# CyrilMorel42/LZ4-JPEG

Hardware: AMD Instinct MI355X
Metric: LZ4 compress GB/s + JPEG DCT Mpixel/s at 1/2/4/8 MI355X; % HBM roofline (higher is better)
Workload: dtype u8

## Files before the change

lz4-jpeg_amd/csrc/lz4r_emit.h:

```cpp
#pragma once
#include "lz4r_layout.h"
#include "wave64.h"

namespace {

constexpr int kGH = 32;
constexpr int kEW = 8;
constexpr int kRecPre = kHeadW;
constexpr int kGSplit = kGT / kGH;
constexpr int kEmitImg = kGH * kBlkOutMax + 32;
constexpr int kStagePad = 16;
constexpr int kStage = kStagePad + kGH * kBlk + 32;
static_assert(kStage < (1 << 16), "stage offsets fit 16 bits");

__device__ __forceinline__ void or_bytes(uint32_t *buf32, int x, uint32_t v) {
  const uint64_t w = (uint64_t)v << (8 * (x & 3));
  atomicOr(&buf32[x >> 2], (uint32_t)w);
  atomicOr(&buf32[(x >> 2) + 1], (uint32_t)(w >> 32));
}

__device__ __forceinline__ void emit_records(const int wv, const int lane, const int h0,
                                             const int h1, const uint64_t G0, const int lead,
                                             const uint64_t *toff, uint8_t *img,
                                             const uint8_t *stage,
                                             const uint32_t (*recst)[kRecPre],
                                             uint32_t (*marks)[64], const uint4 *pmask,
                                             const uint8_t *__restrict__ wovf) {
  {
    constexpr int kBW = kGH / kEW;
    const int bl0 = h0 + wv * kBW, bl1 = min(h1, bl0 + kBW);
    if (bl0 < bl1) {
      uint32_t *const out32 = reinterpret_cast<uint32_t *>(img);
      const int nbk = bl1 - bl0;
      const uint32_t hd = lane < nbk ? recst[bl0 - h0 + lane][0] : 0u;
      const uint32_t ns = hd >> 16;
      const uint32_t sinc = wave_incl_add(ns);
      const int Stot = (int)lane63(sinc);
      const int sst = (int)(sinc - ns);
      int st[kBW];
#pragma unroll
      for (int i = 0; i < kBW; ++i)
        st[i] = i < nbk ? __builtin_amdgcn_readlane(sst, i) : 0x7fffffff;
      int end_prev = 0, wcur = lead + (int)(toff[bl0] - G0) + 3;
      for (int f0 = 0; f0 < Stot; f0 += 64) {
        const int f = f0 + lane;
        const bool valid = f < Stot;
        int bi = 0, sb = 0;
#pragma unroll
        for (int i = 1; i < kBW; ++i) {
          const bool ge = f >= st[i];
          bi += ge ? 1 : 0;
          sb = ge ? st[i] : sb;
        }
        const int k = f - sb;
        const int hb = bl0 + bi;
        const uint32_t *rp = reinterpret_cast<const uint32_t *>(wovf + (hb - h0) * kOvf);
        const uint32_t r =
            !valid ? 0u : (1 + k < kRecPre ? recst[hb - h0][1 + k] : rp[1 + k - kRecPre]);
        const int M = (int)((r >> 9) & 255u), D = (int)(r & 511u);
        const int end = (int)(r >> 19);
        const int cpos = end - M;
        const uint32_t upv = dpp<0x138, 0xf, 0xf>((uint32_t)end);
        const int pend = k == 0 ? 0 : (lane == 0 ? end_prev : (int)upv);
        end_prev = (int)lane63((uint32_t)end);
        const int L = cpos - pend;
        const int rem = (L - 15) & 255;
        const int le = L >= 15 ? (rem == 255 ? 2 : 1) : 0;
        const int mx = (M - 4) & 255;
        const bool mextW = M >= 4 && mx >= 15, mextS = M != 0 && mx >= 15;
        const int bytes = valid ? 5 + le + L + (mextW ? 1 : 0) : 0;
        const uint32_t inc = wave_incl_add((uint32_t)bytes);
        const int o = wcur + 3 * bi + (int)inc - bytes;
        const int ib = o - 3;
        const int ol = o + 3 + le;
        if (valid) {
          const int tl = L >= 15 ? 15 : L;
          const int tm = M == 0 ? 0 : (M >= 19 ? 15 : mx);
          const uint32_t ext = le == 0 ? 0u : (rem == 255 ? 255u : (uint32_t)rem);
          const uint32_t SZ = (uint32_t)(5 + le + L + (mextS ? 1 : 0));
          or_bytes(out32, o, (uint32_t)((tl << 4) | tm) | (SZ << 8) | (ext << 24));
          or_bytes(out32, ol + L, (uint32_t)D | (mextW ? ((uint32_t)(mx - 15) & 255u) << 16 : 0u));
          if (k == 0) {
            const uint32_t bh = recst[hb - h0][0];
            or_bytes(out32, ib, ((bh >> 16) & 255u) | ((((bh & 0xFFFFu) + 3u) & 0xFFFFu) << 8));
          }
        }
        {
          const int cw = valid && L > 0 ? ((ol + L - 1) >> 4) - (ol >> 4) + 1 : 0;
          const uint32_t cinc = wave_incl_add((uint32_t)cw);
          const int C = (int)lane63(cinc);
          const int stw = (int)dpp<0x138, 0xf, 0xf>(cinc);
          const int src = kStagePad + kBlk * (hb - h0) + pend;
          const uint32_t rw = ((uint32_t)((ol >> 4) - stw) & 0xFFFFu) | ((uint32_t)(src - ol) << 16);
          const uint32_t rb = (uint32_t)ol | ((uint32_t)(ol + L) << 16);
          uint32_t carry = 0;
          for (int w0 = 0; w0 < C; w0 += 64) {
            wave_sync();
            marks[wv][lane] = 0u;
            if (cw > 0 && stw >= w0 && stw < w0 + 64) marks[wv][stw - w0] = (uint32_t)lane + 1u;
            wave_sync();
            const uint32_t k1 = max(wave_incl_max(marks[wv][lane]), carry);
            carry = lane63(k1);
            const int gw = w0 + lane;
            const int kr = ((int)k1 - 1) & 63;
            const uint32_t kw = (uint32_t)__shfl((int)rw, kr, 64);
            const uint32_t kb = (uint32_t)__shfl((int)rb, kr, 64);
            if (gw < C) {
              const int t = 16 * ((int)(int16_t)(kw & 0xFFFFu) + gw);
              const int xs = t + ((int)kw >> 16);
              const uint32_t *iw = reinterpret_cast<const uint32_t *>(stage + (xs & ~3));
              const uint32_t d0 = iw[0], d1 = iw[1], d2 = iw[2], d3 = iw[3], d4 = iw[4];
              const uint32_t sh = (uint32_t)xs & 3u;
              const int lb = max((int)(kb & 0xFFFFu) - t, 0), hb = min((int)(kb >> 16) - t, 16);
              const uint4 ml = pmask[lb], mh = pmask[hb];
              const uint32_t v0 = __builtin_amdgcn_alignbyte(d1, d0, sh) & (ml.x ^ mh.x);
              const uint32_t v1 = __builtin_amdgcn_alignbyte(d2, d1, sh) & (ml.y ^ mh.y);
              const uint32_t v2 = __builtin_amdgcn_alignbyte(d3, d2, sh) & (ml.z ^ mh.z);
              const uint32_t v3 = __builtin_amdgcn_alignbyte(d4, d3, sh) & (ml.w ^ mh.w);
              atomicOr(reinterpret_cast<unsigned long long *>(img + t),
                       (unsigned long long)v1 << 32 | v0);
              atomicOr(reinterpret_cast<unsigned long long *>(img + t + 8),
                       (unsigned long long)v3 << 32 | v2);
            }
          }
        }
        wcur += (int)lane63(inc);
      }
    }
  }
}

__device__ __forceinline__ void emit_store(const int tid, const int wv, const int lane,
                                           const uint64_t G0, const uint64_t G1, const int lead,
                                           const uint8_t *img, uint8_t *__restrict__ out) {
  if (G1 <= G0) return;
  const uint64_t F = G0 - (uint64_t)lead;
  uint8_t *const outF = out + F;
  const uint32_t nrel = (uint32_t)(G1 - F);
  const uint32_t c0 = lead ? 1u : 0u, c1 = nrel >> 4;
  for (uint32_t ci = c0 + (uint32_t)tid; ci < c1; ci += 64 * kEW)
    __builtin_nontemporal_store(reinterpret_cast<const u32x4 *>(img)[ci],
                                reinterpret_cast<u32x4 *>(outF + 16u * ci));
  if (wv == kEW - 1 && lane < 32) {
    const uint32_t x = lane < 16 ? (uint32_t)lane : 16u * c1 + (uint32_t)(lane - 16);
    const bool own = lane < 16 ? (c0 && x >= (uint32_t)lead && x < nrel) : (c1 >= c0 && x < nrel);
    if (own) outF[x] = img[x];
  }
}

__global__ __launch_bounds__(64 * kEW) void lz4_emit(
    const uint8_t *__restrict__ in, const uint8_t *__restrict__ heads,
    const uint8_t *__restrict__ ovfs, size_t slot_base,
    const uint32_t *__restrict__ tsz, size_t ntiles, size_t g_first,
    const uint32_t *__restrict__ gsum, const uint64_t *__restrict__ part,
    uint8_t *__restrict__ out, uint64_t cap, int hdr, uint64_t nb_total, uint32_t last_n,
    uint64_t *__restrict__ boff) {
  __shared__ uint64_t toff[kGT + 1];
  __shared__ alignas(16) uint8_t img[kEmitImg];
  __shared__ alignas(16) uint8_t stage[kStage];
  __shared__ uint32_t marks[kEW][64];
  __shared__ uint4 pmask[17];
  __shared__ uint32_t recst[kGH][kRecPre];
  const int tid = threadIdx.x, lane = tid & 63, wv = tid >> 6;
  const uint32_t nwg = (uint32_t)((ntiles - g_first * kGT + kGT - 1) / kGT) * kGSplit;
  const uint32_t per = (nwg + 7) / 8;
  const uint32_t wg = (blockIdx.x & 7u) * per + (blockIdx.x >> 3);
  if (wg >= nwg) return;
  const size_t g = g_first + wg / kGSplit;
  const int h0 = (int)(wg % kGSplit) * kGH;
  const size_t g0 = g * kGT;
  const int nt = (int)min((size_t)kGT, ntiles - g0);
  if (h0 >= nt) return;
  const int h1 = min(nt, h0 + kGH);
  const size_t b0 = g0 + h0;
  const int len = (h1 - h0 - 1) * kBlk + (g0 + h1 == nb_total ? (int)last_n : kBlk);
  const uint8_t *src = in + b0 * kBlk;
  const bool al16 = ((uintptr_t)src & 15) == 0;
  const int n16 = al16 ? len >> 4 : 0;
  uint64_t pt = 0;
  uint32_t gs = 0, tv = 0;
  if (tid < 64) {
    __builtin_amdgcn_s_setprio(3);
    const size_t p = g0 / kPart;
    const size_t gfirst = p * 64;
    gs = (gfirst + tid < g) ? gsum[gfirst + tid] : 0u;
    pt = part[p];
    tv = tid < nt ? tsz[g0 + tid] : 0u;
  }
  constexpr int kPerSlot = kRecPre / 4;
  static_assert(kGH * kPerSlot <= 64 * kEW, "one record load per thread");
  uint4 rv = make_uint4(0, 0, 0, 0);
  const int rhb = tid / kPerSlot, rj = tid % kPerSlot;
  const uint8_t *const wheads = heads + (b0 - slot_base) * (size_t)kHead;
  const uint8_t *const wovf = ovfs + (b0 - slot_base) * (size_t)kOvf;
  if (tid < (h1 - h0) * kPerSlot) {
    const u32x4 t = __builtin_nontemporal_load(reinterpret_cast<const u32x4 *>(wheads) + tid);
    rv = make_uint4(t.x, t.y, t.z, t.w);
  }
  constexpr int kSt16 = (kGH * kBlk) / 16;
  constexpr int kStPer = (kSt16 + 64 * kEW - 1) / (64 * kEW);
  uint4 sv[kStPer];
#pragma unroll
  for (int k = 0; k < kStPer; ++k) {
    const int i = tid + k * 64 * kEW;
    u32x4 t = {0u, 0u, 0u, 0u};
    if (i < n16) t = __builtin_nontemporal_load(reinterpret_cast<const u32x4 *>(src) + i);
    sv[k] = make_uint4(t.x, t.y, t.z, t.w);
  }
  for (int i = tid; i < kEmitImg / 16; i += 64 * kEW)
    reinterpret_cast<uint4 *>(img)[i] = make_uint4(0, 0, 0, 0);
  if (tid < 64) {
    const uint64_t base = pt + lane63(wave_incl_add(gs));
    const uint32_t inc = wave_incl_add(tv);
    toff[tid] = base + inc - tv;
    if (tid == 63) toff[kGT] = base + inc;
    if (h0 == 0 && tid < nt) boff[g0 + tid] = base + inc - tv - (uint64_t)hdr;
  }
  if (hdr && g == 0 && h0 == 0 && tid == 0 && cap > 0) out[0] = (uint8_t)nb_total;
  if (tid < (h1 - h0) * kPerSlot) reinterpret_cast<uint4 *>(&recst[rhb][0])[rj] = rv;
  if (tid < 17) {
    uint32_t m[4];
#pragma unroll
    for (int j = 0; j < 4; ++j) {
      const int n = min(max(tid - 4 * j, 0), 4);
      m[j] = n == 4 ? ~0u : (1u << (8 * n)) - 1u;
    }
    pmask[tid] = make_uint4(m[0], m[1], m[2], m[3]);
  }
  {
    uint8_t *dst = stage + kStagePad;
#pragma unroll
    for (int k = 0; k < kStPer; ++k) {
      const int i = tid + k * 64 * kEW;
      if (i < n16) reinterpret_cast<uint4 *>(dst)[i] = sv[k];
    }
    for (int i = (n16 << 4) + tid; i < len; i += 64 * kEW) dst[i] = src[i];
  }
  __syncthreads();
  __builtin_amdgcn_s_setprio(0);
  const uint64_t G0 = toff[h0];
  const int lead = (int)(((uintptr_t)out + G0) & 15);
  emit_records(wv, lane, h0, h1, G0, lead, toff, img, stage, recst, marks, pmask, wovf);
  __syncthreads();
  emit_store(tid, wv, lane, G0, min(toff[h1], cap), lead, img, out);
}

}
```

Before: 458.6.

## Distribute LZ4 emit sequences across waves by 64-sequence chunks instead of blocks

Emission work used to be split as a fixed group of blocks per wave, with each wave walking its blocks' sequences serially. Now all waves share the global sequence index space and stride over 64-sequence chunks. Each chunk finds its starting block with a ballot/popcount and works out its output offset from the block offset table, plus the chunk's tail prefix. The goal is to balance load when sequence counts differ across blocks. In exchange it adds per-chunk descriptor lookup, marks-based segmenting, and a fallback serial prefix loop for long blocks, which could cost extra work.

```diff
diff --git a/lz4-jpeg_amd/csrc/lz4r_emit.h b/lz4-jpeg_amd/csrc/lz4r_emit.h
--- a/lz4-jpeg_amd/csrc/lz4r_emit.h
+++ b/lz4-jpeg_amd/csrc/lz4r_emit.h
@@ -19,6 +19,20 @@
   atomicOr(&buf32[(x >> 2) + 1], (uint32_t)(w >> 32));
 }
 
+__device__ __forceinline__ uint32_t load_record(const uint32_t (*recst)[kRecPre],
+                                                const uint8_t *__restrict__ wovf, int b, int k) {
+  const uint32_t *rp = reinterpret_cast<const uint32_t *>(wovf + b * kOvf);
+  return 1 + k < kRecPre ? recst[b][1 + k] : rp[1 + k - kRecPre];
+}
+
+__device__ __forceinline__ int sequence_bytes(uint32_t r, int pend) {
+  const int M = (int)((r >> 9) & 255u);
+  const int L = (int)(r >> 19) - M - pend;
+  const int le = L >= 15 ? ((((L - 15) & 255) == 255) ? 2 : 1) : 0;
+  const int mx = (M - 4) & 255;
+  return 5 + le + L + (M >= 4 && mx >= 15 ? 1 : 0);
+}
+
 __device__ __forceinline__ void emit_records(const int wv, const int lane, const int h0,
                                              const int h1, const uint64_t G0, const int lead,
                                              const uint64_t *toff, uint8_t *img,
@@ -26,105 +40,118 @@
                                              const uint32_t (*recst)[kRecPre],
                                              uint32_t (*marks)[64], const uint4 *pmask,
                                              const uint8_t *__restrict__ wovf) {
-  {
-    constexpr int kBW = kGH / kEW;
-    const int bl0 = h0 + wv * kBW, bl1 = min(h1, bl0 + kBW);
-    if (bl0 < bl1) {
-      uint32_t *const out32 = reinterpret_cast<uint32_t *>(img);
-      const int nbk = bl1 - bl0;
-      const uint32_t hd = lane < nbk ? recst[bl0 - h0 + lane][0] : 0u;
-      const uint32_t ns = hd >> 16;
-      const uint32_t sinc = wave_incl_add(ns);
-      const int Stot = (int)lane63(sinc);
-      const int sst = (int)(sinc - ns);
-      int st[kBW];
-#pragma unroll
-      for (int i = 0; i < kBW; ++i)
-        st[i] = i < nbk ? __builtin_amdgcn_readlane(sst, i) : 0x7fffffff;
-      int end_prev = 0, wcur = lead + (int)(toff[bl0] - G0) + 3;
-      for (int f0 = 0; f0 < Stot; f0 += 64) {
-        const int f = f0 + lane;
-        const bool valid = f < Stot;
-        int bi = 0, sb = 0;
-#pragma unroll
-        for (int i = 1; i < kBW; ++i) {
-          const bool ge = f >= st[i];
-          bi += ge ? 1 : 0;
-          sb = ge ? st[i] : sb;
+  uint32_t *const out32 = reinterpret_cast<uint32_t *>(img);
+  const uint32_t ns = lane < h1 - h0 ? recst[lane][0] >> 16 : 0u;
+  const uint32_t sinc = wave_incl_add(ns);
+  const int T = (int)lane63(sinc);
+  const uint32_t sst = sinc - ns;
+  const uint32_t desc = ns ? ((uint32_t)(lane + 1) << 16) | sst : 0u;
+  const int rel = lead - (int)(uint32_t)G0;
+  const int wvu = __builtin_amdgcn_readfirstlane(wv);
+  const uint32_t *const toff32 = reinterpret_cast<const uint32_t *>(toff);
+  for (int f0 = 64 * wvu; f0 < T; f0 += 64 * kEW) {
+    const bool valid = f0 + lane < T;
+    const int cb = __builtin_popcountll(ballot(sst <= (uint32_t)f0)) - 1;
+    const uint32_t cd = (uint32_t)__builtin_amdgcn_readlane((int)desc, cb);
+    const int k0 = f0 - (int)(cd & 0xFFFFu);
+    const int cn = __builtin_amdgcn_readlane((int)sinc, cb) - f0;
+    const int nz = k0 != 0 ? 1 : 0;
+    const uint32_t tb = toff32[2 * (h0 + cb + nz)];
+    uint32_t rprev = recst[cb][min(k0, kRecPre - 1)];
+    wave_sync();
+    marks[wv][lane] = 0u;
+    if (sst - (uint32_t)f0 - 1u < 63u) marks[wv][sst - (uint32_t)f0] = desc;
+    wave_sync();
+    const uint32_t bd = max(wave_incl_max(marks[wv][lane]), cd);
+    const int bi = (int)(bd >> 16) - 1;
+    const int k = f0 + lane - (int)(bd & 0xFFFFu);
+    const int hb = h0 + bi;
+    uint32_t r = recst[bi][min(1 + k, kRecPre - 1)];
+    if (valid && 1 + k >= kRecPre)
+      r = reinterpret_cast<const uint32_t *>(wovf + bi * kOvf)[1 + k - kRecPre];
+    r = valid ? r : 0u;
+    asm volatile("" : "+v"(rprev));
+    if (lane == 0 && k0 >= kRecPre)
+      rprev = reinterpret_cast<const uint32_t *>(wovf + cb * kOvf)[k0 - kRecPre];
+    const int end_prev = k0 != 0 ? (int)(rprev >> 19) : 0;
+    const int M = (int)((r >> 9) & 255u), D = (int)(r & 511u);
+    const int end = (int)(r >> 19);
+    const int cpos = end - M;
+    const uint32_t upv = dpp<0x138, 0xf, 0xf>((uint32_t)end);
+    const int pend = k == 0 ? 0 : (lane == 0 ? end_prev : (int)upv);
+    const int L = cpos - pend;
+    const int rem = (L - 15) & 255;
+    const int le = L >= 15 ? (rem == 255 ? 2 : 1) : 0;
+    const int mx = (M - 4) & 255;
+    const bool mextW = M >= 4 && mx >= 15, mextS = M != 0 && mx >= 15;
+    const int bytes = valid ? 5 + le + L + (mextW ? 1 : 0) : 0;
+    const uint32_t inc = wave_incl_add((uint32_t)bytes);
+    const int tail = __builtin_amdgcn_readlane((int)inc, (cn - 1) & 63);
+    int first = rel + (int)tb + (nz ? -tail : 3);
+    if (nz & (cn > 64 ? 1 : 0)) {
+      int pre = 0, pe = 0;
+      for (int j0 = 0; j0 < k0; j0 += 64) {
+        const int j = j0 + lane;
+        const uint32_t q = j < k0 ? load_record(recst, wovf, cb, j) : 0u;
+        const uint32_t up = dpp<0x138, 0xf, 0xf>(q >> 19);
+        const int qb = j < k0 ? sequence_bytes(q, lane == 0 ? pe : (int)up) : 0;
+        pe = (int)lane63(q >> 19);
+        pre += (int)lane63(wave_incl_add((uint32_t)qb));
+      }
+      first = rel + (int)toff32[2 * (h0 + cb)] + 3 + pre;
+    }
+    const int o = first + 3 * (bi - cb) + (int)inc - bytes;
+    const int ib = o - 3;
+    const int ol = o + 3 + le;
+    if (valid) {
+      const int tl = L >= 15 ? 15 : L;
+      const int tm = M == 0 ? 0 : (M >= 19 ? 15 : mx);
+      const uint32_t ext = le == 0 ? 0u : (rem == 255 ? 255u : (uint32_t)rem);
+      const uint32_t SZ = (uint32_t)(5 + le + L + (mextS ? 1 : 0));
+      or_bytes(out32, o, (uint32_t)((tl << 4) | tm) | (SZ << 8) | (ext << 24));
+      or_bytes(out32, ol + L, (uint32_t)D | (mextW ? ((uint32_t)(mx - 15) & 255u) << 16 : 0u));
+      if (k == 0) {
+        const uint32_t bh = recst[hb - h0][0];
+        or_bytes(out32, ib, ((bh >> 16) & 255u) | ((((bh & 0xFFFFu) + 3u) & 0xFFFFu) << 8));
+      }
+    }
+    {
+      const int cw = valid && L > 0 ? ((ol + L - 1) >> 4) - (ol >> 4) + 1 : 0;
+      const uint32_t cinc = wave_incl_add((uint32_t)cw);
+      const int C = (int)lane63(cinc);
+      const int stw = (int)dpp<0x138, 0xf, 0xf>(cinc);
+      const int src = kStagePad + kBlk * (hb - h0) + pend;
+      const uint32_t rw = ((uint32_t)((ol >> 4) - stw) & 0xFFFFu) | ((uint32_t)(src - ol) << 16);
+      const uint32_t rb = (uint32_t)ol | ((uint32_t)(ol + L) << 16);
+      uint32_t carry = 0;
+      for (int w0 = 0; w0 < C; w0 += 64) {
+        wave_sync();
+        marks[wv][lane] = 0u;
+        if (cw > 0 && stw >= w0 && stw < w0 + 64) marks[wv][stw - w0] = (uint32_t)lane + 1u;
+        wave_sync();
+        const uint32_t k1 = max(wave_incl_max(marks[wv][lane]), carry);
+        carry = lane63(k1);
+        const int gw = w0 + lane;
+        const int kr = ((int)k1 - 1) & 63;
+        const uint32_t kw = (uint32_t)__shfl((int)rw, kr, 64);
+        const uint32_t kb = (uint32_t)__shfl((int)rb, kr, 64);
+        if (gw < C) {
+          const int t = 16 * ((int)(int16_t)(kw & 0xFFFFu) + gw);
+          const int xs = t + ((int)kw >> 16);
+          const uint32_t *iw = reinterpret_cast<const uint32_t *>(stage + (xs & ~3));
+          const uint32_t d0 = iw[0], d1 = iw[1], d2 = iw[2], d3 = iw[3], d4 = iw[4];
+          const uint32_t sh = (uint32_t)xs & 3u;
+          const int lb = max((int)(kb & 0xFFFFu) - t, 0), hb = min((int)(kb >> 16) - t, 16);
+          const uint4 ml = pmask[lb], mh = pmask[hb];
+          const uint32_t v0 = __builtin_amdgcn_alignbyte(d1, d0, sh) & (ml.x ^ mh.x);
+          const uint32_t v1 = __builtin_amdgcn_alignbyte(d2, d1, sh) & (ml.y ^ mh.y);
+          const uint32_t v2 = __builtin_amdgcn_alignbyte(d3, d2, sh) & (ml.z ^ mh.z);
+          const uint32_t v3 = __builtin_amdgcn_alignbyte(d4, d3, sh) & (ml.w ^ mh.w);
+          atomicOr(reinterpret_cast<unsigned long long *>(img + t),
+                   (unsigned long long)v1 << 32 | v0);
+          atomicOr(reinterpret_cast<unsigned long long *>(img + t + 8),
+                   (unsigned long long)v3 << 32 | v2);
         }
-        const int k = f - sb;
-        const int hb = bl0 + bi;
-        const uint32_t *rp = reinterpret_cast<const uint32_t *>(wovf + (hb - h0) * kOvf);
-        const uint32_t r =
-            !valid ? 0u : (1 + k < kRecPre ? recst[hb - h0][1 + k] : rp[1 + k - kRecPre]);
-        const int M = (int)((r >> 9) & 255u), D = (int)(r & 511u);
-        const int end = (int)(r >> 19);
-        const int cpos = end - M;
-        const uint32_t upv = dpp<0x138, 0xf, 0xf>((uint32_t)end);
-        const int pend = k == 0 ? 0 : (lane == 0 ? end_prev : (int)upv);
-        end_prev = (int)lane63((uint32_t)end);
-        const int L = cpos - pend;
-        const int rem = (L - 15) & 255;
-        const int le = L >= 15 ? (rem == 255 ? 2 : 1) : 0;
-        const int mx = (M - 4) & 255;
-        const bool mextW = M >= 4 && mx >= 15, mextS = M != 0 && mx >= 15;
-        const int bytes = valid ? 5 + le + L + (mextW ? 1 : 0) : 0;
-        const uint32_t inc = wave_incl_add((uint32_t)bytes);
-        const int o = wcur + 3 * bi + (int)inc - bytes;
-        const int ib = o - 3;
-        const int ol = o + 3 + le;
-        if (valid) {
-          const int tl = L >= 15 ? 15 : L;
-          const int tm = M == 0 ? 0 : (M >= 19 ? 15 : mx);
-          const uint32_t ext = le == 0 ? 0u : (rem == 255 ? 255u : (uint32_t)rem);
-          const uint32_t SZ = (uint32_t)(5 + le + L + (mextS ? 1 : 0));
-          or_bytes(out32, o, (uint32_t)((tl << 4) | tm) | (SZ << 8) | (ext << 24));
-          or_bytes(out32, ol + L, (uint32_t)D | (mextW ? ((uint32_t)(mx - 15) & 255u) << 16 : 0u));
-          if (k == 0) {
-            const uint32_t bh = recst[hb - h0][0];
-            or_bytes(out32, ib, ((bh >> 16) & 255u) | ((((bh & 0xFFFFu) + 3u) & 0xFFFFu) << 8));
-          }
-        }
-        {
-          const int cw = valid && L > 0 ? ((ol + L - 1) >> 4) - (ol >> 4) + 1 : 0;
-          const uint32_t cinc = wave_incl_add((uint32_t)cw);
-          const int C = (int)lane63(cinc);
-          const int stw = (int)dpp<0x138, 0xf, 0xf>(cinc);
-          const int src = kStagePad + kBlk * (hb - h0) + pend;
-          const uint32_t rw = ((uint32_t)((ol >> 4) - stw) & 0xFFFFu) | ((uint32_t)(src - ol) << 16);
-          const uint32_t rb = (uint32_t)ol | ((uint32_t)(ol + L) << 16);
-          uint32_t carry = 0;
-          for (int w0 = 0; w0 < C; w0 += 64) {
-            wave_sync();
-            marks[wv][lane] = 0u;
-            if (cw > 0 && stw >= w0 && stw < w0 + 64) marks[wv][stw - w0] = (uint32_t)lane + 1u;
-            wave_sync();
-            const uint32_t k1 = max(wave_incl_max(marks[wv][lane]), carry);
-            carry = lane63(k1);
-            const int gw = w0 + lane;
-            const int kr = ((int)k1 - 1) & 63;
-            const uint32_t kw = (uint32_t)__shfl((int)rw, kr, 64);
-            const uint32_t kb = (uint32_t)__shfl((int)rb, kr, 64);
-            if (gw < C) {
-              const int t = 16 * ((int)(int16_t)(kw & 0xFFFFu) + gw);
-              const int xs = t + ((int)kw >> 16);
-              const uint32_t *iw = reinterpret_cast<const uint32_t *>(stage + (xs & ~3));
-              const uint32_t d0 = iw[0], d1 = iw[1], d2 = iw[2], d3 = iw[3], d4 = iw[4];
-              const uint32_t sh = (uint32_t)xs & 3u;
-              const int lb = max((int)(kb & 0xFFFFu) - t, 0), hb = min((int)(kb >> 16) - t, 16);
-              const uint4 ml = pmask[lb], mh = pmask[hb];
-              const uint32_t v0 = __builtin_amdgcn_alignbyte(d1, d0, sh) & (ml.x ^ mh.x);
-              const uint32_t v1 = __builtin_amdgcn_alignbyte(d2, d1, sh) & (ml.y ^ mh.y);
-              const uint32_t v2 = __builtin_amdgcn_alignbyte(d3, d2, sh) & (ml.z ^ mh.z);
-              const uint32_t v3 = __builtin_amdgcn_alignbyte(d4, d3, sh) & (ml.w ^ mh.w);
-              atomicOr(reinterpret_cast<unsigned long long *>(img + t),
-                       (unsigned long long)v1 << 32 | v0);
-              atomicOr(reinterpret_cast<unsigned long long *>(img + t + 8),
-                       (unsigned long long)v3 << 32 | v2);
-            }
-          }
-        }
-        wcur += (int)lane63(inc);
       }
     }
   }
```

Result: faster. 464.9 (median of 6 runs) (+1.4%).
